# cloneofsimo/paint-with-words-sd

Hardware: NVIDIA H100
Metric: unet_steps_per_sec_512sq_cfg (higher is better)
Workload: dtype f16

## Files before the change

### include/pww_b200.h

```cpp
#ifndef PWW_B200_H_
#define PWW_B200_H_

#include <stddef.h>
#include <stdint.h>

#ifdef __cplusplus
extern "C" {
#endif

typedef enum {
  PWW_OK = 0,
  PWW_ERR_BAD_ARG = -1,
  PWW_ERR_UNSUPPORTED = -2,
  PWW_ERR_CUDA = -3,
  PWW_ERR_WORKSPACE = -4
} pww_status_t;

#define PWW_STAT_MAX 0
#define PWW_STAT_STD 1

int pww_version(void);

const char* pww_status_str(int status);

// ... 45 lines not shown
int pww_xattn_fused_bf16(const void* q, const void* k, const void* v, void* out,
                         int B, int H, int N, int T, int D,
                         int64_t q_batch_stride, int64_t q_row_stride,
                         int64_t k_batch_stride, int64_t k_row_stride,
                         int64_t o_batch_stride, int64_t o_row_stride,
                         const void* mpack, int64_t mpack_batch_stride, int Bw, const int8_t* cidx,
                         const int32_t* wmap_index, int stat, const float* g_sigma, float scale,
                         float* stats, void* workspace, size_t workspace_bytes, void* stream);

int pww_xattn_stats_multi_f16(const void* q, const void* k,
                              int B, int H, int N, int T, int D,
                              int64_t q_batch_stride, int64_t q_row_stride,
                              int64_t k_batch_stride, int64_t k_row_stride,
                              const int32_t* stat, const int32_t* wmap_index,
                              float* stats ,
                              void* workspace, size_t workspace_bytes, void* stream);
int pww_xattn_fwd_multi_f16(const void* q, const void* k, const void* v, void* out,
                            int B, int H, int N, int T, int D,
                            int64_t q_batch_stride, int64_t q_row_stride,
                            int64_t k_batch_stride, int64_t k_row_stride,
                            int64_t o_batch_stride, int64_t o_row_stride,
                            const float* wmap, int64_t wmap_batch_stride, const int32_t* wmap_index,
                            const float* stats, const float* g_sigma, float scale, void* stream);
int pww_xattn_fused_multi_f16(const void* q, const void* k, const void* v, void* out,
                              int B, int H, int N, int T, int D,
                              int64_t q_batch_stride, int64_t q_row_stride,
                              int64_t k_batch_stride, int64_t k_row_stride,
                              int64_t o_batch_stride, int64_t o_row_stride,
                              const void* mpack, int64_t mpack_batch_stride, int Bw, const int8_t* cidx,
                              const int32_t* wmap_index, const int32_t* stat, const float* g_sigma, float scale,
                              float* stats, void* workspace, size_t workspace_bytes, void* stream);
int pww_xattn_stats_multi_bf16(const void* q, const void* k,
                               int B, int H, int N, int T, int D,
                               int64_t q_batch_stride, int64_t q_row_stride,
                               int64_t k_batch_stride, int64_t k_row_stride,
                               const int32_t* stat, const int32_t* wmap_index,
                               float* stats ,
                               void* workspace, size_t workspace_bytes, void* stream);
int pww_xattn_fwd_multi_bf16(const void* q, const void* k, const void* v, void* out,
                             int B, int H, int N, int T, int D,
                             int64_t q_batch_stride, int64_t q_row_stride,
                             int64_t k_batch_stride, int64_t k_row_stride,
                             int64_t o_batch_stride, int64_t o_row_stride,
                             const float* wmap, int64_t wmap_batch_stride, const int32_t* wmap_index,
                             const float* stats, const float* g_sigma, float scale, void* stream);
int pww_xattn_fused_multi_bf16(const void* q, const void* k, const void* v, void* out,
                               int B, int H, int N, int T, int D,
                               int64_t q_batch_stride, int64_t q_row_stride,
                               int64_t k_batch_stride, int64_t k_row_stride,
                               int64_t o_batch_stride, int64_t o_row_stride,
                               const void* mpack, int64_t mpack_batch_stride, int Bw, const int8_t* cidx,
                               const int32_t* wmap_index, const int32_t* stat, const float* g_sigma, float scale,
                               float* stats, void* workspace, size_t workspace_bytes, void* stream);

int pww_xattn_fused_rec_f16(const void* q, const void* k, const void* v, void* out,
                            int B, int H, int N, int T, int D,
                            int64_t q_batch_stride, int64_t q_row_stride,
                            int64_t k_batch_stride, int64_t k_row_stride,
                            int64_t o_batch_stride, int64_t o_row_stride,
                            const void* mpack, int64_t mpack_batch_stride, int Bw, const int8_t* cidx,
                            const int32_t* wmap_index, const int32_t* stat, const float* g_sigma, float scale,
                            float* stats, void* workspace, size_t workspace_bytes, void* stream,
                            const int8_t* ridx, const int32_t* rec_index, float* rec_acc, int64_t rec_batch_stride);
int pww_xattn_fused_rec_bf16(const void* q, const void* k, const void* v, void* out,
                             int B, int H, int N, int T, int D,
                             int64_t q_batch_stride, int64_t q_row_stride,
                             int64_t k_batch_stride, int64_t k_row_stride,
                             int64_t o_batch_stride, int64_t o_row_stride,
                             const void* mpack, int64_t mpack_batch_stride, int Bw, const int8_t* cidx,
                             const int32_t* wmap_index, const int32_t* stat, const float* g_sigma, float scale,
                             float* stats, void* workspace, size_t workspace_bytes, void* stream,
                             const int8_t* ridx, const int32_t* rec_index, float* rec_acc, int64_t rec_batch_stride);

int pww_attn_fwd_f16(const void* q, const void* k, const void* v, void* out,
                     int B, int H, int N, int D,
                     int64_t qkv_batch_stride, int64_t qkv_row_stride,
                     int64_t o_batch_stride, int64_t o_row_stride,
                     float scale, void* stream);
int pww_attn_fwd_bf16(const void* q, const void* k, const void* v, void* out,
                      int B, int H, int N, int D,
                      int64_t qkv_batch_stride, int64_t qkv_row_stride,
                      int64_t o_batch_stride, int64_t o_row_stride,
                      float scale, void* stream);

size_t pww_groupnorm_workspace_bytes(int B, int HW, int G);
int pww_groupnorm_nhwc_f16(const void* x, const void* add, int64_t add_batch_stride ,
                           const void* gamma, const void* beta, void* y,
                           int B, int HW, int C, int G, float eps, int silu,
                           void* workspace, size_t workspace_bytes, void* stream);
int pww_groupnorm_nhwc_bf16(const void* x, const void* add, int64_t add_batch_stride ,
                            const void* gamma, const void* beta, void* y,
                            int B, int HW, int C, int G, float eps, int silu,
                            void* workspace, size_t workspace_bytes, void* stream);

int pww_geglu_f16(const void* in, void* out, int64_t M, int I, void* stream);
int pww_geglu_bf16(const void* in, void* out, int64_t M, int I, void* stream);

int pww_add_layernorm_f16(const void* x, const void* res, const void* gamma, const void* beta, void* sum_out, void* y,
                          int64_t M, int C, float eps, void* stream);
int pww_add_layernorm_bf16(const void* x, const void* res, const void* gamma, const void* beta, void* sum_out, void* y,
                           int64_t M, int C, float eps, void* stream);

int pww_resnet_residual_f16(const void* a, const void* h, const float* bias, void* out, int64_t rows, int C,
                            void* stream);
int pww_resnet_residual_bf16(const void* a, const void* h, const float* bias, void* out, int64_t rows, int C,
                             void* stream);

#define PWW_DTYPE_F32 0
#define PWW_DTYPE_F16 1
#define PWW_DTYPE_BF16 4
int pww_sampler_input(const float* latents, const float* scale, const float* extra, void* out, int out_dtype,
                      int m, int channels, int height, int width, void* stream);
int pww_sampler_update(const void* eps, int eps_dtype, int64_t eps_batch_stride, int64_t eps_channel_stride,
                       int64_t eps_row_stride, int64_t eps_col_stride,
                       float* latents, float* history, int history_len, const float* noise,
                       const float* guidance, const float* beta, const float* form,
                       int m, int height, int width, void* stream);

int pww_control_inject_f16(int n, void* const* dst, const void* const* res, const int64_t* elems_per_image, int rows,
                           const float* scales, void* stream);
int pww_control_inject_bf16(int n, void* const* dst, const void* const* res, const int64_t* elems_per_image, int rows,
                            const float* scales, void* stream);

int pww_control_combine_f16(int units, int n, void* const* out, const void* const* res,
                            const int64_t* elems_per_image, int rows, const float* scales, void* stream);
int pww_control_combine_bf16(int units, int n, void* const* out, const void* const* res,
                             const int64_t* elems_per_image, int rows, const float* scales, void* stream);

#ifdef __cplusplus
}
#endif
#endif
```

### paint_with_words_sd_b200/_native.py

```python
from __future__ import annotations

import ctypes
import os
from typing import Optional

import torch

_HERE = os.path.dirname(os.path.abspath(__file__))
LIB_PATH = os.environ.get("PWW_B200_LIB", os.path.join(_HERE, "libpww_b200.so"))

PWW_STAT_MAX, PWW_STAT_STD = 0, 1
PWW_DTYPE_F32, PWW_DTYPE_F16, PWW_DTYPE_BF16 = 0, 1, 4

EXPORTS = (
    "pww_version", "pww_status_str", "pww_last_cuda_error", "pww_device_supported",
    "pww_xattn_workspace_bytes", "pww_xattn_stats_f16", "pww_xattn_fwd_f16", "pww_attn_fwd_f16",
    "pww_xattn_fused_workspace_bytes", "pww_xattn_fused_f16",
    "pww_xattn_stats_multi_f16", "pww_xattn_fwd_multi_f16", "pww_xattn_fused_multi_f16",
    "pww_groupnorm_workspace_bytes", "pww_groupnorm_nhwc_f16", "pww_geglu_f16", "pww_add_layernorm_f16",
    "pww_sampler_input", "pww_sampler_update",
    "pww_xattn_stats_bf16", "pww_xattn_fwd_bf16", "pww_xattn_fused_bf16",
    "pww_xattn_stats_multi_bf16", "pww_xattn_fwd_multi_bf16", "pww_xattn_fused_multi_bf16",
    "pww_attn_fwd_bf16", "pww_groupnorm_nhwc_bf16", "pww_geglu_bf16", "pww_add_layernorm_bf16",
    "pww_control_inject_f16", "pww_control_inject_bf16",
    "pww_control_combine_f16", "pww_control_combine_bf16",
    "pww_resnet_residual_f16", "pww_resnet_residual_bf16",
    "pww_xattn_fused_rec_f16", "pww_xattn_fused_rec_bf16",
)


class NativeError(RuntimeError):
    pass


_lib: Optional[ctypes.CDLL] = None
launch_count = 0


def lib() -> ctypes.CDLL:
    global _lib
    if _lib is not None:
        return _lib
    if not os.path.exists(LIB_PATH):
        raise NativeError(
            f"{LIB_PATH} not found: build it with `python -m paint_with_words_sd_b200.csrc.build` "
            "(there is no CPU / PyTorch fallback for the attention path)")
    L = ctypes.CDLL(LIB_PATH)
    c_i, c_i64, c_vp, c_f, c_sz = ctypes.c_int, ctypes.c_int64, ctypes.c_void_p, ctypes.c_float, ctypes.c_size_t
    L.pww_version.restype = c_i
    L.pww_status_str.restype = ctypes.c_char_p
    L.pww_status_str.argtypes = [c_i]
    L.pww_last_cuda_error.restype = ctypes.c_char_p
    L.pww_device_supported.restype = c_i
    L.pww_xattn_workspace_bytes.restype = c_sz
    L.pww_xattn_workspace_bytes.argtypes = [c_i] * 5
    L.pww_xattn_stats_f16.restype = c_i
    L.pww_xattn_stats_f16.argtypes = [c_vp, c_vp, c_i, c_i, c_i, c_i, c_i, c_i64, c_i64, c_i64, c_i64, c_i, c_vp,
                                      c_vp, c_vp, c_sz, c_vp]
    L.pww_xattn_fwd_f16.restype = c_i
    L.pww_xattn_fwd_f16.argtypes = [c_vp, c_vp, c_vp, c_vp, c_i, c_i, c_i, c_i, c_i, c_i64, c_i64, c_i64, c_i64,
                                    c_i64, c_i64, c_vp, c_i64, c_vp, c_vp, c_vp, c_f, c_vp]
    L.pww_xattn_fused_workspace_bytes.restype = c_sz
    L.pww_xattn_fused_workspace_bytes.argtypes = []
    L.pww_xattn_fused_f16.restype = c_i
    L.pww_xattn_fused_f16.argtypes = [c_vp, c_vp, c_vp, c_vp, c_i, c_i, c_i, c_i, c_i, c_i64, c_i64, c_i64, c_i64,
                                      c_i64, c_i64, c_vp, c_i64, c_i, c_vp, c_vp, c_i, c_vp, c_f, c_vp, c_vp, c_sz, c_vp]
    L.pww_xattn_stats_multi_f16.restype = c_i
    L.pww_xattn_stats_multi_f16.argtypes = [c_vp, c_vp, c_i, c_i, c_i, c_i, c_i, c_i64, c_i64, c_i64, c_i64, c_vp, c_vp,
                                            c_vp, c_vp, c_sz, c_vp]
    L.pww_xattn_fwd_multi_f16.restype = c_i
    L.pww_xattn_fwd_multi_f16.argtypes = list(L.pww_xattn_fwd_f16.argtypes)
    L.pww_xattn_fused_multi_f16.restype = c_i
    L.pww_xattn_fused_multi_f16.argtypes = [c_vp, c_vp, c_vp, c_vp, c_i, c_i, c_i, c_i, c_i, c_i64, c_i64, c_i64, c_i64,
                                            c_i64, c_i64, c_vp, c_i64, c_i, c_vp, c_vp, c_vp, c_vp, c_f, c_vp, c_vp, c_sz,
                                            c_vp]
    L.pww_xattn_fused_rec_f16.restype = c_i
    L.pww_xattn_fused_rec_f16.argtypes = list(L.pww_xattn_fused_multi_f16.argtypes) + [c_vp, c_vp, c_vp, c_i64]
    L.pww_attn_fwd_f16.restype = c_i
    L.pww_attn_fwd_f16.argtypes = [c_vp, c_vp, c_vp, c_vp, c_i, c_i, c_i, c_i, c_i64, c_i64, c_i64, c_i64, c_f, c_vp]
    L.pww_groupnorm_workspace_bytes.restype = c_sz
    L.pww_groupnorm_workspace_bytes.argtypes = [c_i, c_i, c_i]
    L.pww_groupnorm_nhwc_f16.restype = c_i
    L.pww_groupnorm_nhwc_f16.argtypes = [c_vp, c_vp, c_i64, c_vp, c_vp, c_vp, c_i, c_i, c_i, c_i, c_f, c_i, c_vp, c_sz, c_vp]
    L.pww_geglu_f16.restype = c_i
    L.pww_geglu_f16.argtypes = [c_vp, c_vp, c_i64, c_i, c_vp]
    L.pww_add_layernorm_f16.restype = c_i
    L.pww_add_layernorm_f16.argtypes = [c_vp, c_vp, c_vp, c_vp, c_vp, c_vp, c_i64, c_i, c_f, c_vp]
    L.pww_resnet_residual_f16.restype = c_i
    L.pww_resnet_residual_f16.argtypes = [c_vp, c_vp, c_vp, c_vp, c_i64, c_i, c_vp]
    L.pww_control_inject_f16.restype = c_i
    L.pww_control_inject_f16.argtypes = [c_i, ctypes.POINTER(c_vp), ctypes.POINTER(c_vp), ctypes.POINTER(c_i64), c_i,
                                         c_vp, c_vp]
    L.pww_control_combine_f16.restype = c_i
    L.pww_control_combine_f16.argtypes = [c_i, c_i, ctypes.POINTER(c_vp), ctypes.POINTER(c_vp), ctypes.POINTER(c_i64),
                                          c_i, c_vp, c_vp]
    for name in EXPORTS:
        if name.endswith("_bf16"):
            twin = getattr(L, name[:-len("_bf16")] + "_f16")
            fn = getattr(L, name)
            fn.restype, fn.argtypes = twin.restype, list(twin.argtypes)
    L.pww_sampler_input.restype = c_i
    L.pww_sampler_input.argtypes = [c_vp, c_vp, c_vp, c_vp, c_i, c_i, c_i, c_i, c_i, c_vp]
    L.pww_sampler_update.restype = c_i
    L.pww_sampler_update.argtypes = [c_vp, c_i, c_i64, c_i64, c_i64, c_i64, c_vp, c_vp, c_i, c_vp, c_vp, c_vp, c_vp,
                                     c_i, c_i, c_i, c_vp]
    _lib = L
    return L


def entry(name: str, dtype):
    return getattr(lib(), name + ("_bf16" if dtype == torch.bfloat16 else "_f16"))


def check(status: int, what: str) -> None:
    if status != 0:
        L = lib()
        msg = L.pww_status_str(status).decode()
        if status == -3:
            msg += ": " + L.pww_last_cuda_error().decode()
        raise NativeError(f"{what} failed: {msg} (status {status})")
```

### paint_with_words_sd_b200/csrc/mma_sm90.cuh

```cuda
#pragma once
#include <cuda_runtime.h>
#include <stdint.h>

#include <type_traits>

#include "pww_common.cuh"

namespace pww {
namespace ptx {

__device__ __forceinline__ uint32_t smem_u32(const void* p) { return (uint32_t)__cvta_generic_to_shared(p); }

__device__ __forceinline__ void cp_async16(uint32_t dst, const void* src, uint32_t src_bytes) {
  asm volatile("cp.async.cg.shared.global [%0], [%1], 16, %2;" ::"r"(dst), "l"(src), "r"(src_bytes) : "memory");
}
__device__ __forceinline__ void cp_async_commit() { asm volatile("cp.async.commit_group;" ::: "memory"); }
template <int N>
__device__ __forceinline__ void cp_async_wait() { asm volatile("cp.async.wait_group %0;" ::"n"(N) : "memory"); }

__device__ __forceinline__ void ldsm_x4(uint32_t addr, uint32_t& r0, uint32_t& r1, uint32_t& r2, uint32_t& r3) {
  asm volatile("ldmatrix.sync.aligned.m8n8.x4.shared.b16 {%0, %1, %2, %3}, [%4];"
               : "=r"(r0), "=r"(r1), "=r"(r2), "=r"(r3) : "r"(addr));
}
__device__ __forceinline__ void ldsm_x4_t(uint32_t addr, uint32_t& r0, uint32_t& r1, uint32_t& r2, uint32_t& r3) {
  asm volatile("ldmatrix.sync.aligned.m8n8.x4.trans.shared.b16 {%0, %1, %2, %3}, [%4];"
               : "=r"(r0), "=r"(r1), "=r"(r2), "=r"(r3) : "r"(addr));
}
__device__ __forceinline__ void ldsm_x2_t(uint32_t addr, uint32_t& r0, uint32_t& r1) {
  asm volatile("ldmatrix.sync.aligned.m8n8.x2.trans.shared.b16 {%0, %1}, [%2];" : "=r"(r0), "=r"(r1) : "r"(addr));
}

template <typename E>
__device__ __forceinline__ void mma16816(float* c, const uint32_t* a, uint32_t b0, uint32_t b1) {
  static_assert(std::is_same_v<E, __half> || std::is_same_v<E, __nv_bfloat16>, "fp16 or bf16 operands");
  if constexpr (std::is_same_v<E, __half>) {
    asm volatile(
        "mma.sync.aligned.m16n8k16.row.col.f32.f16.f16.f32 {%0, %1, %2, %3}, {%4, %5, %6, %7}, {%8, %9}, "
        "{%0, %1, %2, %3};"
        : "+f"(c[0]), "+f"(c[1]), "+f"(c[2]), "+f"(c[3])
        : "r"(a[0]), "r"(a[1]), "r"(a[2]), "r"(a[3]), "r"(b0), "r"(b1));
  } else {
    asm volatile(
        "mma.sync.aligned.m16n8k16.row.col.f32.bf16.bf16.f32 {%0, %1, %2, %3}, {%4, %5, %6, %7}, {%8, %9}, "
        "{%0, %1, %2, %3};"
        : "+f"(c[0]), "+f"(c[1]), "+f"(c[2]), "+f"(c[3])
        : "r"(a[0]), "r"(a[1]), "r"(a[2]), "r"(a[3]), "r"(b0), "r"(b1));
  }
}

__device__ __forceinline__ float ex2(float x) {
  float y;
  asm("ex2.approx.ftz.f32 %0, %1;" : "=f"(y) : "f"(x));
  return y;
}
template <typename E>
__device__ __forceinline__ uint32_t pack2(float lo, float hi) {
  const typename Elem<E>::E2 h = Elem<E>::from_float2(lo, hi);
  return *reinterpret_cast<const uint32_t*>(&h);
}
template <typename E>
__device__ __forceinline__ float2 unpack2(uint32_t v) {
  return Elem<E>::to_float2(*reinterpret_cast<const typename Elem<E>::E2*>(&v));
}
__device__ __forceinline__ unsigned long long ld_acquire_gpu_u64(const unsigned long long* p) {
  unsigned long long v;
  asm volatile("ld.acquire.gpu.global.u64 %0, [%1];" : "=l"(v) : "l"(p) : "memory");
  return v;
}

}
}
```

### paint_with_words_sd_b200/csrc/pww_abi.cu

```cuda
#include <stdio.h>
#include <string.h>

#include "pww_common.cuh"
#include "xattn_tc.cuh"
#include "xattn_fused2.cuh"
#include "attn_tc.cuh"
#include "unet_ops.cuh"
#include "sampler_step.cuh"
#include "control_inject.cuh"
#include "control_combine.cuh"
#include <stdlib.h>
#include <algorithm>
#include <type_traits>

namespace {

thread_local char g_last_cuda_error[640] = "";

int cuda_fail(cudaError_t e);

bool aligned16(const void* p) { return (reinterpret_cast<uintptr_t>(p) & 15u) == 0; }

bool supported_head_dim(int D) { return D == 40 || D == 64 || D == 80 || D == 160; }

int check_common(const void* q, const void* k, int B, int H, int N, int T, int D, int64_t q_bs, int64_t q_rs,
                 int64_t k_bs, int64_t k_rs) {
  if (!q || !k || B <= 0 || H <= 0 || N <= 0 || T <= 0 || D <= 0) return PWW_ERR_BAD_ARG;
  if (!aligned16(q) || !aligned16(k)) return PWW_ERR_BAD_ARG;
  if ((q_bs | q_rs | k_bs | k_rs) & 7) return PWW_ERR_BAD_ARG;
  if (q_rs < (int64_t)H * D || k_rs < (int64_t)H * D) return PWW_ERR_BAD_ARG;
  if (!supported_head_dim(D) || !pww::core::supported_keys(T)) return PWW_ERR_UNSUPPORTED;
  return PWW_OK;
}

template <int D_, int KC_>
struct Shape {
  static constexpr int D = D_, KC = KC_;
};
template <int D, typename F>
cudaError_t with_chunks(int T, F&& f) {
  switch (pww::core::chunks_of(T)) {
    case 1: return f(Shape<D, 1>{});
    case 2: return f(Shape<D, 2>{});
    case 3: return f(Shape<D, 3>{});
  }
  return cudaErrorInvalidValue;
}
template <typename F>
cudaError_t with_shape(int D, int T, F&& f) {
  switch (D) {
    case 40: return with_chunks<40>(T, f);
    case 64: return with_chunks<64>(T, f);
    case 80: return with_chunks<80>(T, f);
    case 160: return with_chunks<160>(T, f);
  }
  return cudaErrorInvalidValue;
}

template <int lo, int hi, typename F>
void with_int(int v, F&& f) {
  if constexpr (lo < hi)
    if (v != lo) return with_int<lo + 1, hi>(v, f);
  f(std::integral_constant<int, lo>{});
}

size_t align_up(size_t x, size_t a) { return (x + a - 1) / a * a; }

constexpr int kStatSlotsPerImage = 2048;

int cuda_fail(cudaError_t e) {
  snprintf(g_last_cuda_error, sizeof(g_last_cuda_error), "%s: %s ", cudaGetErrorName(e), cudaGetErrorString(e));
  return PWW_ERR_CUDA;
}

template <typename E>
pww::XattnParams<E> xattn_params(const void* q, const void* k, const void* v, void* out, int B, int H, int N, int T, int D,
                                 int64_t q_bs, int64_t q_rs, int64_t k_bs, int64_t k_rs, int64_t o_bs, int64_t o_rs) {
  pww::XattnParams<E> p;
  memset(&p, 0, sizeof(p));
  p.q = (const E*)q; p.k = (const E*)k; p.v = (const E*)v; p.out = (E*)out;
  p.B = B; p.H = H; p.N = N; p.T = T; p.D = D;
  p.q_bs = q_bs; p.q_rs = q_rs; p.k_bs = k_bs; p.k_rs = k_rs; p.o_bs = o_bs; p.o_rs = o_rs;
  return p;
}

template <typename E>
pww::XattnParams<E> images(const pww::XattnParams<E>& p, int b0, int n) {
  pww::XattnParams<E> c = p;
  c.B = n;
// ... 163 lines not shown
  if (!x || !gamma || !beta || !y || !workspace || B <= 0 || HW <= 0 || C <= 0 || G <= 0) return PWW_ERR_BAD_ARG;
  if (!aligned16(x) || !aligned16(y) || !aligned16(gamma) || !aligned16(beta) || (add && !aligned16(add)))
    return PWW_ERR_BAD_ARG;
  if ((C & 7) || (C % G) || G > 64 || (C >> 3) > 1024) return PWW_ERR_UNSUPPORTED;
  if (add && ((add_batch_stride & 7) || add_batch_stride < C)) return PWW_ERR_BAD_ARG;
  if (workspace_bytes < pww_groupnorm_workspace_bytes(B, HW, G)) return PWW_ERR_WORKSPACE;
  const pww::uops::GnSplit sp = pww::uops::gn_split(HW, C, G);
  pww::uops::GnParams<E> p;
  p.x = (const E*)x; p.add = (const E*)add; p.add_bs = add_batch_stride; p.gamma = (const E*)gamma; p.beta = (const E*)beta;
  p.y = (E*)y;
  p.partial = (float2*)workspace;
  p.HW = HW; p.C = C; p.G = G; p.eps = eps; p.silu = silu;
  p.sv = sp.sv; p.chunks = sp.chunks; p.rows_per_chunk = sp.rows_per_chunk;
  cudaStream_t s = (cudaStream_t)stream;
  const size_t smem1 = (64 + (size_t)2 * sp.rpp * sp.sv * 8) * sizeof(float);
  if (smem1 > 48 * 1024) {
    const cudaError_t e = pww::allow_dynamic_smem<pww::uops::gn_stats_kernel<E>>(64 * 1024 + 256);
    if (e != cudaSuccess) return cuda_fail(e);
  }
  pww::uops::gn_stats_kernel<E><<<dim3(sp.chunks, sp.slices, B), sp.threads, smem1, s>>>(p);
  int rows = 4;
  while (rows > 1 && (long long)B * sp.slices * pww::ceil_div(HW, sp.rpp * rows) < 2 * pww::num_sms()) rows >>= 1;
  cudaLaunchAttribute pdl;
  pdl.id = cudaLaunchAttributeProgrammaticStreamSerialization;
  pdl.val.programmaticStreamSerializationAllowed = 1;
  cudaLaunchConfig_t cfg = {};
  cfg.gridDim = dim3(pww::ceil_div(HW, sp.rpp * rows), sp.slices, B);
  cfg.blockDim = dim3(sp.threads);
  cfg.stream = s;
  cfg.attrs = &pdl;
  cfg.numAttrs = 1;
  cudaError_t e = cudaLaunchKernelEx(&cfg, pww::uops::gn_apply_kernel<E>, p, sp.rpp * rows);
  if (e == cudaSuccess) e = cudaGetLastError();
  return e == cudaSuccess ? PWW_OK : cuda_fail(e);
}

template <typename E>
int geglu(const void* in, void* out, int64_t M, int I, void* stream) {
  if (!in || !out || M <= 0 || I <= 0 || !aligned16(in) || !aligned16(out)) return PWW_ERR_BAD_ARG;
  if (I & 7) return PWW_ERR_UNSUPPORTED;
  const long long total = (long long)M * (I >> 3);
  long long blocks = (total + 255) / 256;
  const long long cap = (long long)pww::num_sms() * 16;
  if (blocks > cap) blocks = cap;
  pww::uops::geglu_kernel<E><<<(int)blocks, 256, 0, (cudaStream_t)stream>>>((const E*)in, (E*)out, M, I);
  cudaError_t e = cudaGetLastError();
  return e == cudaSuccess ? PWW_OK : cuda_fail(e);
}

template <typename E>
int add_layernorm(const void* x, const void* res, const void* gamma, const void* beta, void* sum_out, void* y, int64_t M,
                  int C, float eps, void* stream) {
  if (!x || !gamma || !beta || !y || M <= 0 || C <= 0) return PWW_ERR_BAD_ARG;
  if (!aligned16(x) || !aligned16(y) || !aligned16(gamma) || !aligned16(beta) || (res && !aligned16(res)) ||
      (sum_out && !aligned16(sum_out)))
    return PWW_ERR_BAD_ARG;
  if ((C & 7) || C > 2048) return PWW_ERR_UNSUPPORTED;
  const int warps = 8;
  const unsigned grid = (unsigned)((M + warps - 1) / warps);
  with_int<1, 8>(((C >> 3) + 31) / 32, [&](auto vpl) {
    pww::uops::add_layernorm_kernel<E, vpl><<<grid, warps * 32, 0, (cudaStream_t)stream>>>(
        (const E*)x, (const E*)res, (const E*)gamma, (const E*)beta, (E*)sum_out, (E*)y, M, C, eps);
  });
  cudaError_t e = cudaGetLastError();
  return e == cudaSuccess ? PWW_OK : cuda_fail(e);
}

template <typename E>
int resnet_residual(const void* a, const void* h, const float* bias, void* out, int64_t rows, int C, void* stream) {
  if (!a || !h || !bias || !out || rows <= 0 || C <= 0 || (C & 7)) return PWW_ERR_BAD_ARG;
  if (!aligned16(a) || !aligned16(h) || !aligned16(bias) || !aligned16(out)) return PWW_ERR_BAD_ARG;
  const long long total = (long long)rows * (C >> 3);
  long long blocks = (total + 255) / 256;
  const long long cap = (long long)pww::num_sms() * 16;
  if (blocks > cap) blocks = cap;
  pww::uops::resnet_residual_kernel<E><<<(int)blocks, 256, 0, (cudaStream_t)stream>>>(
      (const E*)a, (const E*)h, bias, (E*)out, total, C >> 3);
  cudaError_t e = cudaGetLastError();
  return e == cudaSuccess ? PWW_OK : cuda_fail(e);
}

template <typename E>
int attn_fwd(const void* q,const void* k, const void* v, void* out, int B, int H, int N, int D, int64_t qkv_batch_stride,
             int64_t qkv_row_stride, int64_t o_batch_stride, int64_t o_row_stride, float scale, void* stream) {
  if (!q || !k || !v || !out || B <= 0 || H <= 0 || N <= 0 || D <= 0) return PWW_ERR_BAD_ARG;
  if (!aligned16(q) || !aligned16(k) || !aligned16(v) || !aligned16(out)) return PWW_ERR_BAD_ARG;
  if ((qkv_batch_stride | qkv_row_stride | o_batch_stride | o_row_stride) & 7) return PWW_ERR_BAD_ARG;
  if (qkv_row_stride < (int64_t)H * D || o_row_stride < (int64_t)H * D) return PWW_ERR_BAD_ARG;
  if (!supported_head_dim(D)) return PWW_ERR_UNSUPPORTED;
  const cudaError_t e = with_shape(D, 1, [&](auto sh) {
    return pww::fa::launch<sh.D, E>(q, k, v, out, B, H, N, qkv_batch_stride, qkv_row_stride, o_batch_stride,
                                    o_row_stride, scale, (cudaStream_t)stream);
  });
  return e == cudaSuccess ? PWW_OK : cuda_fail(e);
}

template <typename E>
int control_inject(int n, void* const* dst, const void* const* res, const int64_t* elems_per_image, int rows,
                   const float* scales, void* stream) {
  if (n < 1 || n > pww::ctl::kMaxLevels || rows < 1 || !dst || !res || !elems_per_image) return PWW_ERR_BAD_ARG;
  pww::ctl::InjectArgs a;
  a.off[0] = 0;
  for (int k = 0; k < n; ++k) {
    const int64_t e = elems_per_image[k];
    if (e <= 0 || (e % pww::ctl::kVec) != 0) return PWW_ERR_BAD_ARG;
    if (!dst[k] || !res[k] || !aligned16(dst[k]) || !aligned16(res[k])) return PWW_ERR_BAD_ARG;
    a.dst[k] = dst[k];
    a.res[k] = res[k];
    a.vec_per_image[k] = e / pww::ctl::kVec;
    a.off[k + 1] = a.off[k] + (int64_t)rows * a.vec_per_image[k];
  }
  for (int k = n; k < pww::ctl::kMaxLevels; ++k) {
    a.dst[k] = nullptr;
    a.res[k] = nullptr;
    a.vec_per_image[k] = 0;
    a.off[k + 1] = a.off[n];
  }
  a.scales = scales;
  a.n = n;
  a.rows = rows;
  const cudaError_t e = pww::ctl::launch_inject<E>(a, (int64_t)pww::num_sms() * 8, (cudaStream_t)stream);
  return e == cudaSuccess ? PWW_OK : cuda_fail(e);
}

template <typename E>
int control_combine(int units, int n, void* const* out, const void* const* res, const int64_t* elems_per_image,
                    int rows, const float* scales, void* stream) {
  if (units < 1 || units > pww::ctl::kMaxUnits || n < 1 || n > pww::ctl::kMaxLevels || rows < 1 || !out || !res ||
      !elems_per_image || !scales)
    return PWW_ERR_BAD_ARG;
  pww::ctl::CombineArgs a = {};
  for (int k = 0; k < n; ++k) {
    const int64_t e = elems_per_image[k];
    if (e <= 0 || (e % pww::ctl::kVec) != 0) return PWW_ERR_BAD_ARG;
    if (!out[k] || !aligned16(out[k])) return PWW_ERR_BAD_ARG;
    a.out[k] = out[k];
    a.vec_per_image[k] = e / pww::ctl::kVec;
    a.off[k + 1] = a.off[k] + (int64_t)rows * a.vec_per_image[k];
  }
  for (int i = 0; i < units * n; ++i) {
    if (!res[i] || !aligned16(res[i])) return PWW_ERR_BAD_ARG;
    a.res[i] = res[i];
  }
  for (int k = n; k < pww::ctl::kMaxLevels; ++k) a.off[k + 1] = a.off[n];
  a.scales = scales;
  a.units = units;
  a.n = n;
  a.rows = rows;
  const cudaError_t e = pww::ctl::launch_combine<E>(a, (int64_t)pww::num_sms() * 8, (cudaStream_t)stream);
  return e == cudaSuccess ? PWW_OK : cuda_fail(e);
}

}

extern "C" {

int pww_xattn_stats_f16(const void* q, const void* k, int B, int H, int N, int T, int D, int64_t q_batch_stride,
    int64_t q_row_stride, int64_t k_batch_stride, int64_t k_row_stride, int stat, const int32_t* wmap_index,
    float* stats, void* workspace, size_t workspace_bytes, void* stream) {
  return xattn_stats<__half>(
      q, k, B, H, N, T, D, q_batch_stride, q_row_stride, k_batch_stride, k_row_stride, stat, nullptr, false,
      wmap_index, stats, workspace, workspace_bytes, stream);
}
int pww_xattn_stats_bf16(const void* q, const void* k, int B, int H, int N, int T, int D, int64_t q_batch_stride,
    int64_t q_row_stride, int64_t k_batch_stride, int64_t k_row_stride, int stat, const int32_t* wmap_index,
    float* stats, void* workspace, size_t workspace_bytes, void* stream) {
  return xattn_stats<__nv_bfloat16>(
      q, k, B, H, N, T, D, q_batch_stride, q_row_stride, k_batch_stride, k_row_stride, stat, nullptr, false,
      wmap_index, stats, workspace, workspace_bytes, stream);
}

int pww_xattn_stats_multi_f16(const void* q, const void* k, int B, int H, int N, int T, int D, int64_t q_batch_stride,
// ... 40 lines not shown
    const float* g_sigma, float scale, void* stream) {
  return xattn_fwd<__nv_bfloat16>(
      q, k, v, out, B, H, N, T, D, q_batch_stride, q_row_stride, k_batch_stride, k_row_stride,
      o_batch_stride, o_row_stride, wmap, wmap_batch_stride, wmap_index, stats, g_sigma, 1, scale, stream);
}

size_t pww_xattn_fused_workspace_bytes(void) { return pww::fx::fused_workspace_bytes(); }

int pww_xattn_fused_f16(const void* q, const void* k, const void* v, void* out, int B, int H, int N, int T, int D,
    int64_t q_batch_stride, int64_t q_row_stride, int64_t k_batch_stride, int64_t k_row_stride, int64_t o_batch_stride,
    int64_t o_row_stride, const void* mpack, int64_t mpack_batch_stride, int Bw, const int8_t* cidx,
    const int32_t* wmap_index, int stat, const float* g_sigma, float scale, float* stats, void* workspace,
    size_t workspace_bytes, void* stream) {
  return xattn_fused<__half>(q, k, v, out, B, H, N, T, D, q_batch_stride, q_row_stride, k_batch_stride, k_row_stride,
      o_batch_stride, o_row_stride, mpack, mpack_batch_stride, Bw, cidx, wmap_index, stat, nullptr, false,
      g_sigma, scale, stats, workspace, workspace_bytes, stream);
}
int pww_xattn_fused_bf16(const void* q, const void* k, const void* v, void* out, int B, int H, int N, int T, int D,
    int64_t q_batch_stride, int64_t q_row_stride, int64_t k_batch_stride, int64_t k_row_stride, int64_t o_batch_stride,
    int64_t o_row_stride, const void* mpack, int64_t mpack_batch_stride, int Bw, const int8_t* cidx,
    const int32_t* wmap_index, int stat, const float* g_sigma, float scale, float* stats, void* workspace,
    size_t workspace_bytes, void* stream) {
  return xattn_fused<__nv_bfloat16>(
      q, k, v, out, B, H, N, T, D, q_batch_stride, q_row_stride, k_batch_stride, k_row_stride,
      o_batch_stride, o_row_stride, mpack, mpack_batch_stride, Bw, cidx, wmap_index, stat, nullptr, false,
      g_sigma, scale, stats, workspace, workspace_bytes, stream);
}

int pww_xattn_fused_multi_f16(const void* q, const void* k, const void* v, void* out, int B, int H, int N, int T, int D,
    int64_t q_batch_stride, int64_t q_row_stride, int64_t k_batch_stride, int64_t k_row_stride, int64_t o_batch_stride,
    int64_t o_row_stride, const void* mpack, int64_t mpack_batch_stride, int Bw, const int8_t* cidx,
    const int32_t* wmap_index, const int32_t* stat, const float* g_sigma, float scale, float* stats, void* workspace,
    size_t workspace_bytes, void* stream) {
  return xattn_fused<__half>(q, k, v, out, B, H, N, T, D, q_batch_stride, q_row_stride, k_batch_stride, k_row_stride,
      o_batch_stride, o_row_stride, mpack, mpack_batch_stride, Bw, cidx, wmap_index, PWW_STAT_MAX, stat, true,
      g_sigma, scale, stats, workspace, workspace_bytes, stream);
}
int pww_xattn_fused_multi_bf16(const void* q, const void* k, const void* v, void* out, int B, int H, int N, int T, int D,
    int64_t q_batch_stride, int64_t q_row_stride, int64_t k_batch_stride, int64_t k_row_stride, int64_t o_batch_stride,
    int64_t o_row_stride, const void* mpack, int64_t mpack_batch_stride, int Bw, const int8_t* cidx,
    const int32_t* wmap_index, const int32_t* stat, const float* g_sigma, float scale, float* stats, void* workspace,
    size_t workspace_bytes, void* stream) {
  return xattn_fused<__nv_bfloat16>(
      q, k, v, out, B, H, N, T, D, q_batch_stride, q_row_stride, k_batch_stride, k_row_stride,
      o_batch_stride, o_row_stride, mpack, mpack_batch_stride, Bw, cidx, wmap_index, PWW_STAT_MAX, stat, true,
      g_sigma, scale, stats, workspace, workspace_bytes, stream);
}

int pww_xattn_fused_rec_f16(const void* q, const void* k, const void* v, void* out, int B, int H, int N, int T, int D,
    int64_t q_batch_stride, int64_t q_row_stride, int64_t k_batch_stride, int64_t k_row_stride, int64_t o_batch_stride,
    int64_t o_row_stride, const void* mpack, int64_t mpack_batch_stride, int Bw, const int8_t* cidx,
    const int32_t* wmap_index, const int32_t* stat, const float* g_sigma, float scale, float* stats, void* workspace,
    size_t workspace_bytes, void* stream, const int8_t* ridx, const int32_t* rec_index, float* rec_acc,
    int64_t rec_batch_stride) {
  const pww::fx::FxRecord rec = {ridx, rec_index, rec_acc, rec_batch_stride};
  return xattn_fused<__half>(q, k, v, out, B, H, N, T, D, q_batch_stride, q_row_stride, k_batch_stride, k_row_stride,
      o_batch_stride, o_row_stride, mpack, mpack_batch_stride, Bw, cidx, wmap_index, PWW_STAT_MAX, stat, true,
      g_sigma, scale, stats, workspace, workspace_bytes, stream, &rec);
}
int pww_xattn_fused_rec_bf16(const void* q, const void* k, const void* v, void* out, int B, int H, int N, int T, int D,
    int64_t q_batch_stride, int64_t q_row_stride, int64_t k_batch_stride, int64_t k_row_stride, int64_t o_batch_stride,
    int64_t o_row_stride, const void* mpack, int64_t mpack_batch_stride, int Bw, const int8_t* cidx,
    const int32_t* wmap_index, const int32_t* stat, const float* g_sigma, float scale, float* stats, void* workspace,
    size_t workspace_bytes, void* stream, const int8_t* ridx, const int32_t* rec_index, float* rec_acc,
    int64_t rec_batch_stride) {
  const pww::fx::FxRecord rec = {ridx, rec_index, rec_acc, rec_batch_stride};
  return xattn_fused<__nv_bfloat16>(
      q, k, v, out, B, H, N, T, D, q_batch_stride, q_row_stride, k_batch_stride, k_row_stride,
      o_batch_stride, o_row_stride, mpack, mpack_batch_stride, Bw, cidx, wmap_index, PWW_STAT_MAX, stat, true,
      g_sigma, scale, stats, workspace, workspace_bytes, stream, &rec);
}

int pww_attn_fwd_f16(const void* q, const void* k, const void* v, void* out, int B, int H, int N, int D,
    int64_t qkv_batch_stride, int64_t qkv_row_stride, int64_t o_batch_stride, int64_t o_row_stride, float scale,
    void* stream) {
  return attn_fwd<__half>(
      q, k, v, out, B, H, N, D, qkv_batch_stride, qkv_row_stride, o_batch_stride, o_row_stride, scale, stream);
}
int pww_attn_fwd_bf16(const void* q, const void* k, const void* v, void* out, int B, int H, int N, int D,
    int64_t qkv_batch_stride, int64_t qkv_row_stride, int64_t o_batch_stride, int64_t o_row_stride, float scale,
    void* stream) {
  return attn_fwd<__nv_bfloat16>(
      q, k, v, out, B, H, N, D, qkv_batch_stride, qkv_row_stride, o_batch_stride, o_row_stride, scale, stream);
}

size_t pww_groupnorm_workspace_bytes(int B, int HW, int G) {
  if (B <= 0 || HW <= 0 || G <= 0) return 0;
  const size_t chunks = (size_t)std::min(HW, pww::uops::kGnMaxChunks);
  return align_up((size_t)B * G * chunks * sizeof(float2), 256);
}

int pww_groupnorm_nhwc_f16(const void* x, const void* add, int64_t add_batch_stride, const void* gamma,
    const void* beta, void* y, int B, int HW, int C, int G, float eps, int silu, void* workspace, size_t workspace_bytes,
    void* stream) {
  return groupnorm_nhwc<__half>(
      x, add, add_batch_stride, gamma, beta, y, B, HW, C, G, eps, silu, workspace, workspace_bytes,
      stream);
}
int pww_groupnorm_nhwc_bf16(const void* x, const void* add, int64_t add_batch_stride, const void* gamma,
    const void* beta, void* y, int B, int HW, int C, int G, float eps, int silu, void* workspace, size_t workspace_bytes,
    void* stream) {
  return groupnorm_nhwc<__nv_bfloat16>(
      x, add, add_batch_stride, gamma, beta, y, B, HW, C, G, eps, silu, workspace, workspace_bytes,
      stream);
}

int pww_geglu_f16(const void* in, void* out, int64_t M, int I, void* stream) {
  return geglu<__half>(in, out, M, I, stream);
}
int pww_geglu_bf16(const void* in, void* out, int64_t M, int I, void* stream) {
  return geglu<__nv_bfloat16>(in, out, M, I, stream);
}

int pww_add_layernorm_f16(const void* x, const void* res, const void* gamma, const void* beta, void* sum_out, void* y,
    int64_t M, int C, float eps, void* stream) {
  return add_layernorm<__half>(x, res, gamma, beta, sum_out, y, M, C, eps, stream);
}
int pww_add_layernorm_bf16(const void* x, const void* res, const void* gamma, const void* beta, void* sum_out, void* y,
    int64_t M, int C, float eps, void* stream) {
  return add_layernorm<__nv_bfloat16>(x, res, gamma, beta, sum_out, y, M, C, eps, stream);
}

int pww_resnet_residual_f16(const void* a, const void* h, const float* bias, void* out, int64_t rows, int C,
                            void* stream) {
  return resnet_residual<__half>(a, h, bias, out, rows, C, stream);
}
int pww_resnet_residual_bf16(const void* a, const void* h, const float* bias, void* out, int64_t rows, int C,
                             void* stream) {
  return resnet_residual<__nv_bfloat16>(a, h, bias, out, rows, C, stream);
}

int pww_sampler_input(const float* latents, const float* scale, const float* extra, void* out, int out_dtype, int m,
                      int channels, int height, int width, void* stream) {
  if (!latents || !scale || !out || m <= 0 || height <= 0 || width <= 0) return PWW_ERR_BAD_ARG;
  if (channels != 4 && channels != 9) return PWW_ERR_BAD_ARG;
  if ((channels == 9) != (extra != nullptr)) return PWW_ERR_BAD_ARG;
  if (out_dtype != PWW_DTYPE_F32 && out_dtype != PWW_DTYPE_F16 && out_dtype != PWW_DTYPE_BF16) return PWW_ERR_UNSUPPORTED;
  pww::smp::InputArgs a;
  a.lat = latents; a.scale = scale; a.extra = extra; a.out = out; a.m = m; a.C = channels; a.hw = height * width;
  const bool px4 = (a.hw % 4) == 0 && aligned16(latents) && (!extra || aligned16(extra)) && aligned16(out);
  cudaStream_t s = (cudaStream_t)stream;
  const cudaError_t e = out_dtype == PWW_DTYPE_F16    ? pww::smp::launch_input<__half>(a, px4, s)
                        : out_dtype == PWW_DTYPE_BF16 ? pww::smp::launch_input<__nv_bfloat16>(a, px4, s)
                                                      : pww::smp::launch_input<float>(a, px4, s);
  return e == cudaSuccess ? PWW_OK : cuda_fail(e);
}

int pww_sampler_update(const void* eps, int eps_dtype, int64_t eps_batch_stride, int64_t eps_channel_stride,
                       int64_t eps_row_stride, int64_t eps_col_stride, float* latents, float* history, int history_len,
                       const float* noise, const float* guidance, const float* beta, const float* form, int m,
                       int height, int width, void* stream) {
  if (!eps || !latents || !history || !guidance || !beta || !form) return PWW_ERR_BAD_ARG;
  if (m <= 0 || height <= 0 || width <= 0 || history_len < 1 || history_len > 4) return PWW_ERR_BAD_ARG;
  if (eps_dtype != PWW_DTYPE_F32 && eps_dtype != PWW_DTYPE_F16 && eps_dtype != PWW_DTYPE_BF16) return PWW_ERR_UNSUPPORTED;
  pww::smp::UpdateArgs a;
  a.eps = eps; a.e_sn = eps_batch_stride; a.e_sc = eps_channel_stride; a.e_sh = eps_row_stride; a.e_sw = eps_col_stride;
  a.lat = latents; a.hist = history; a.noise = noise; a.gscale = guidance; a.beta = beta; a.form = form;
  a.m = m; a.h = height; a.w = width; a.nh = history_len;
  const int64_t hw = (int64_t)height * width;
  const size_t es = eps_dtype == PWW_DTYPE_F32 ? 4 : 2;
  const bool px4 = (hw % 4) == 0 && aligned16(latents) && aligned16(history) && (!noise || aligned16(noise));
  const size_t need = px4 ? 16 : 4 * es;
  const bool cl = eps_channel_stride == 1 && eps_col_stride == 4 && eps_row_stride == 4 * (int64_t)width &&
                  (reinterpret_cast<uintptr_t>(eps) % need) == 0 && ((size_t)eps_batch_stride * es) % need == 0;
  cudaStream_t s = (cudaStream_t)stream;
  const cudaError_t e = eps_dtype == PWW_DTYPE_F16    ? pww::smp::launch_update<__half>(a, px4, cl, s)
// ... 48 lines not shown
```

Baseline: 159.8.

## Add Hopper wgmma flash-attention kernel for head dim 40 self-attention

Adds an SM90 self-attention kernel that uses warpgroup wgmma for QK^T (shared-memory operands) and for PV (register operands), with a 3-stage cp.async K/V pipeline. Each CTA runs two warpgroups handling 128 query rows. An extra padded chunk whose V column is set to one makes the PV product also produce the softmax row sum. The kernel is the default for D=40, and the old mma.sync path stays reachable through new _mma entry points. The goal is higher tensor-core throughput for the 64x64 UNet self-attention. The risk is that D=40 pads K to 48 and wastes MMA work, and every wgmma is waited on synchronously, so MMA work does not overlap with softmax.

```diff
diff --git a/include/pww_b200.h b/include/pww_b200.h
--- a/include/pww_b200.h
+++ b/include/pww_b200.h
@@ -151,6 +151,16 @@
                       int64_t qkv_batch_stride, int64_t qkv_row_stride,
                       int64_t o_batch_stride, int64_t o_row_stride,
                       float scale, void* stream);
+int pww_attn_fwd_mma_f16(const void* q, const void* k, const void* v, void* out,
+                         int B, int H, int N, int D,
+                         int64_t qkv_batch_stride, int64_t qkv_row_stride,
+                         int64_t o_batch_stride, int64_t o_row_stride,
+                         float scale, void* stream);
+int pww_attn_fwd_mma_bf16(const void* q, const void* k, const void* v, void* out,
+                          int B, int H, int N, int D,
+                          int64_t qkv_batch_stride, int64_t qkv_row_stride,
+                          int64_t o_batch_stride, int64_t o_row_stride,
+                          float scale, void* stream);
 
 size_t pww_groupnorm_workspace_bytes(int B, int HW, int G);
 int pww_groupnorm_nhwc_f16(const void* x, const void* add, int64_t add_batch_stride ,
diff --git a/paint_with_words_sd_b200/_native.py b/paint_with_words_sd_b200/_native.py
--- a/paint_with_words_sd_b200/_native.py
+++ b/paint_with_words_sd_b200/_native.py
@@ -26,6 +26,7 @@
     "pww_control_combine_f16", "pww_control_combine_bf16",
     "pww_resnet_residual_f16", "pww_resnet_residual_bf16",
     "pww_xattn_fused_rec_f16", "pww_xattn_fused_rec_bf16",
+    "pww_attn_fwd_mma_f16", "pww_attn_fwd_mma_bf16",
 )
 
 
@@ -78,6 +79,8 @@
     L.pww_xattn_fused_rec_f16.argtypes = list(L.pww_xattn_fused_multi_f16.argtypes) + [c_vp, c_vp, c_vp, c_i64]
     L.pww_attn_fwd_f16.restype = c_i
     L.pww_attn_fwd_f16.argtypes = [c_vp, c_vp, c_vp, c_vp, c_i, c_i, c_i, c_i, c_i64, c_i64, c_i64, c_i64, c_f, c_vp]
+    L.pww_attn_fwd_mma_f16.restype = c_i
+    L.pww_attn_fwd_mma_f16.argtypes = list(L.pww_attn_fwd_f16.argtypes)
     L.pww_groupnorm_workspace_bytes.restype = c_sz
     L.pww_groupnorm_workspace_bytes.argtypes = [c_i, c_i, c_i]
     L.pww_groupnorm_nhwc_f16.restype = c_i
diff --git a/paint_with_words_sd_b200/csrc/attn_wgmma.cuh b/paint_with_words_sd_b200/csrc/attn_wgmma.cuh
--- /dev/null
+++ b/paint_with_words_sd_b200/csrc/attn_wgmma.cuh
@@ -0,0 +1,199 @@
+#pragma once
+#include "attn_tc.cuh"
+#include "mma_sm90.cuh"
+#include "pww_common.cuh"
+
+namespace pww {
+namespace fa90 {
+
+constexpr int kD = 40;
+constexpr int kDataChunks = kD / 8;
+constexpr int kChunks = kDataChunks + 1;
+constexpr int kWarpgroups = 2;
+constexpr int kThreads = kWarpgroups * 128;
+constexpr int kBM = 64 * kWarpgroups;
+constexpr int kBN = 128;
+constexpr int kStages = 3;
+static_assert(kBM == kBN, "Q, K and V tiles share one shape");
+constexpr uint32_t kSlab = kBN * 16;
+constexpr uint32_t kTileBytes = kChunks * kSlab;
+constexpr uint32_t kOffKV = kTileBytes;
+constexpr uint32_t kSmem = kTileBytes + kStages * 2 * kTileBytes;
+static_assert(2 * kSmem <= 232448, "two CTAs per SM");
+
+constexpr int kPieces = kBN * kDataChunks;
+constexpr int kSlots = (kPieces + kThreads - 1) / kThreads;
+struct Pieces {
+  uint32_t soff[kSlots];
+  int64_t goff[kSlots];
+};
+
+__device__ __forceinline__ Pieces make_pieces(int64_t rs) {
+  Pieces pc;
+#pragma unroll
+  for (int i = 0; i < kSlots; ++i) {
+    const int idx = threadIdx.x + i * kThreads, r = idx / kDataChunks, c = idx - r * kDataChunks;
+    pc.soff[i] = c * kSlab + r * 16;
+    pc.goff[i] = r * rs + c * 8;
+  }
+  return pc;
+}
+
+template <typename E>
+__device__ __forceinline__ void load_tile(const Pieces& pc, uint32_t dst, const E* src, int valid) {
+#pragma unroll
+  for (int i = 0; i < kSlots; ++i) {
+    if (i == kSlots - 1 && threadIdx.x + i * kThreads >= kPieces) break;
+    const bool ok = (int)((pc.soff[i] & (kSlab - 1)) >> 4) < valid;
+    ptx::cp_async16(dst + pc.soff[i], ok ? (const void*)(src + pc.goff[i]) : (const void*)src, ok ? 16u : 0u);
+  }
+}
+
+template <typename E>
+__global__ void __launch_bounds__(kThreads, 2) attn_fwd_wgmma_kernel(const fa::Params<E> p) {
+  extern __shared__ __align__(128) unsigned char smem[];
+  const uint32_t smem0 = ptx::smem_u32(smem);
+  const int tid = threadIdx.x, wg = tid >> 7, warp = tid >> 5, lane = tid & 31;
+  const int qtiles = (p.N + kBM - 1) / kBM;
+  const int bh = blockIdx.x / qtiles, qt = blockIdx.x - bh * qtiles;
+  const int b = bh / p.H, h = bh - b * p.H;
+  const int row_base = qt * kBM;
+  const int64_t head = (int64_t)b * p.bs + h * kD;
+  const int ntiles = (p.N + kBN - 1) / kBN;
+
+  {
+    const uint32_t one = std::is_same_v<E, __half> ? 0x3C00u : 0x3F80u;
+    for (int i = tid; i < (1 + 2 * kStages) * kBN; i += kThreads) {
+      const int t = i / kBN, r = i - t * kBN;
+      const uint32_t tile = t == 0 ? 0u : kOffKV + (uint32_t)(t - 1) * kTileBytes;
+      const bool is_v = t > 0 && ((t - 1) & 1);
+      *reinterpret_cast<uint4*>(smem + tile + kDataChunks * kSlab + r * 16) = make_uint4(is_v ? one : 0u, 0u, 0u, 0u);
+    }
+  }
+  const Pieces pc = make_pieces(p.rs);
+  auto issue_kv = [&](int j) {
+    if (j < ntiles) {
+      const uint32_t st = smem0 + kOffKV + (uint32_t)(j % kStages) * 2 * kTileBytes;
+      const int rows = p.N - j * kBN < kBN ? p.N - j * kBN : kBN;
+      load_tile(pc, st, p.k + head + (int64_t)j * kBN * p.rs, rows);
+      load_tile(pc, st + kTileBytes, p.v + head + (int64_t)j * kBN * p.rs, rows);
+    }
+    ptx::cp_async_commit();
+  };
+  load_tile(pc, smem0, p.q + head + (int64_t)row_base * p.rs, p.N - row_base < kBM ? p.N - row_base : kBM);
+  issue_kv(0);
+  issue_kv(1);
+
+  float o[24];
+#pragma unroll
+  for (int i = 0; i < 24; ++i) o[i] = 0.f;
+  float m0 = -INFINITY, m1 = -INFINITY;
+  const float sl2 = p.scale * 1.4426950408889634f;
+  const uint32_t qs = smem0 + (uint32_t)wg * 64 * 16;
+#pragma unroll 1
+  for (int jt = 0; jt < ntiles; ++jt) {
+    ptx::cp_async_wait<1>();
+    ptx::fence_proxy_async();
+    __syncthreads();
+    issue_kv(jt + 2);
+    const uint32_t ks = smem0 + kOffKV + (uint32_t)(jt % kStages) * 2 * kTileBytes, vs = ks + kTileBytes;
+
+    float s[64];
+    ptx::wgmma_fence();
+    ptx::wgmma_m64n128k16_ss<E, false>(s, ptx::gmma_desc(qs, kSlab, 16 * 8), ptx::gmma_desc(ks, kSlab, 16 * 8));
+#pragma unroll
+    for (int kk = 1; kk < 3; ++kk)
+      ptx::wgmma_m64n128k16_ss<E, true>(s, ptx::gmma_desc(qs + kk * 2 * kSlab, kSlab, 16 * 8),
+                                        ptx::gmma_desc(ks + kk * 2 * kSlab, kSlab, 16 * 8));
+    ptx::wgmma_commit();
+    ptx::wgmma_wait<0>();
+#pragma unroll
+    for (int i = 0; i < 64; ++i) ptx::reg_fence(s[i]);
+
+    const int kv = p.N - jt * kBN;
+    if (kv < kBN) {
+#pragma unroll
+      for (int i = 0; i < 64; ++i)
+        if (8 * (i >> 2) + 2 * (lane & 3) + (i & 1) >= kv) s[i] = -INFINITY;
+    }
+    float t0 = -INFINITY, t1 = -INFINITY;
+#pragma unroll
+    for (int j = 0; j < 16; ++j) {
+      t0 = fmaxf(t0, fmaxf(s[4 * j], s[4 * j + 1]));
+      t1 = fmaxf(t1, fmaxf(s[4 * j + 2], s[4 * j + 3]));
+    }
+    t0 = fmaxf(t0, __shfl_xor_sync(0xffffffffu, t0, 1));
+    t0 = fmaxf(t0, __shfl_xor_sync(0xffffffffu, t0, 2));
+    t1 = fmaxf(t1, __shfl_xor_sync(0xffffffffu, t1, 1));
+    t1 = fmaxf(t1, __shfl_xor_sync(0xffffffffu, t1, 2));
+    const float mn0 = fmaxf(m0, t0), mn1 = fmaxf(m1, t1);
+    const float a0 = ptx::ex2((m0 - mn0) * sl2), a1 = ptx::ex2((m1 - mn1) * sl2);
+    m0 = mn0; m1 = mn1;
+    const float n0 = -mn0 * sl2, n1 = -mn1 * sl2;
+    uint32_t pa[8][4];
+#pragma unroll
+    for (int j = 0; j < 16; ++j) {
+      pa[j >> 1][(j & 1) * 2] = ptx::pack2<E>(ptx::ex2(fmaf(s[4 * j], sl2, n0)), ptx::ex2(fmaf(s[4 * j + 1], sl2, n0)));
+      pa[j >> 1][(j & 1) * 2 + 1] =
+          ptx::pack2<E>(ptx::ex2(fmaf(s[4 * j + 2], sl2, n1)), ptx::ex2(fmaf(s[4 * j + 3], sl2, n1)));
+    }
+#pragma unroll
+    for (int j = 0; j < 6; ++j) {
+      o[4 * j] *= a0; o[4 * j + 1] *= a0; o[4 * j + 2] *= a1; o[4 * j + 3] *= a1;
+    }
+#pragma unroll
+    for (int i = 0; i < 24; ++i) ptx::reg_fence(o[i]);
+#pragma unroll
+    for (int kk = 0; kk < 8; ++kk)
+#pragma unroll
+      for (int e = 0; e < 4; ++e) ptx::reg_fence(pa[kk][e]);
+    ptx::wgmma_fence();
+#pragma unroll
+    for (int kk = 0; kk < 8; ++kk)
+      ptx::wgmma_m64n48k16_rs<E>(o, pa[kk], ptx::gmma_desc(vs + kk * 2 * 128, 128, kSlab));
+    ptx::wgmma_commit();
+    ptx::wgmma_wait<0>();
+#pragma unroll
+    for (int i = 0; i < 24; ++i) ptx::reg_fence(o[i]);
+#pragma unroll
+    for (int kk = 0; kk < 8; ++kk)
+#pragma unroll
+      for (int e = 0; e < 4; ++e) ptx::reg_fence(pa[kk][e]);
+  }
+
+  const float i0 = 1.f / __shfl_sync(0xffffffffu, o[20], lane & ~3);
+  const float i1 = 1.f / __shfl_sync(0xffffffffu, o[22], lane & ~3);
+  __syncthreads();
+  const int g = lane >> 2, q = lane & 3, r0 = warp * 16 + g;
+#pragma unroll
+  for (int j = 0; j < kDataChunks; ++j) {
+    *reinterpret_cast<uint32_t*>(smem + j * kSlab + r0 * 16 + q * 4) = ptx::pack2<E>(o[4 * j] * i0, o[4 * j + 1] * i0);
+    *reinterpret_cast<uint32_t*>(smem + j * kSlab + (r0 + 8) * 16 + q * 4) =
+        ptx::pack2<E>(o[4 * j + 2] * i1, o[4 * j + 3] * i1);
+  }
+  __syncwarp();
+  E* ob = p.out + (int64_t)b * p.o_bs + h * kD;
+  for (int idx = lane; idx < 16 * kDataChunks; idx += 32) {
+    const int r = idx / kDataChunks, c = idx - r * kDataChunks, row = row_base + warp * 16 + r;
+    if (row < p.N)
+      *reinterpret_cast<uint4*>(ob + (int64_t)row * p.o_rs + c * 8) =
+          *reinterpret_cast<const uint4*>(smem + c * kSlab + (warp * 16 + r) * 16);
+  }
+}
+
+template <typename E>
+cudaError_t launch(const void* q, const void* k, const void* v, void* out, int B, int H, int N, int64_t bs, int64_t rs,
+                   int64_t o_bs, int64_t o_rs, float scale, cudaStream_t s) {
+  fa::Params<E> p;
+  p.q = (const E*)q; p.k = (const E*)k; p.v = (const E*)v; p.out = (E*)out;
+  p.B = B; p.H = H; p.N = N; p.bs = bs; p.rs = rs; p.o_bs = o_bs; p.o_rs = o_rs; p.scale = scale;
+  const cudaError_t e = allow_dynamic_smem<attn_fwd_wgmma_kernel<E>>(kSmem);
+  if (e != cudaSuccess) return e;
+  const long long grid = (long long)B * H * ((N + kBM - 1) / kBM);
+  if (grid > 0x7fffffffLL) return cudaErrorInvalidConfiguration;
+  attn_fwd_wgmma_kernel<E><<<(unsigned)grid, kThreads, kSmem, s>>>(p);
+  return cudaGetLastError();
+}
+
+}
+}
diff --git a/paint_with_words_sd_b200/csrc/mma_sm90.cuh b/paint_with_words_sd_b200/csrc/mma_sm90.cuh
--- a/paint_with_words_sd_b200/csrc/mma_sm90.cuh
+++ b/paint_with_words_sd_b200/csrc/mma_sm90.cuh
@@ -48,6 +48,55 @@
   }
 }
 
+__device__ __forceinline__ uint64_t gmma_desc(uint32_t smem_addr, uint32_t lbo, uint32_t sbo) {
+  return (uint64_t)((smem_addr & 0x3FFFFu) >> 4) | ((uint64_t)((lbo >> 4) & 0x3FFFu) << 16) |
+         ((uint64_t)((sbo >> 4) & 0x3FFFu) << 32);
+}
+__device__ __forceinline__ void fence_proxy_async() { asm volatile("fence.proxy.async.shared::cta;" ::: "memory"); }
+__device__ __forceinline__ void wgmma_fence() { asm volatile("wgmma.fence.sync.aligned;" ::: "memory"); }
+__device__ __forceinline__ void wgmma_commit() { asm volatile("wgmma.commit_group.sync.aligned;" ::: "memory"); }
+template <int N>
+__device__ __forceinline__ void wgmma_wait() { asm volatile("wgmma.wait_group.sync.aligned %0;" ::"n"(N) : "memory"); }
+__device__ __forceinline__ void reg_fence(float& r) { asm volatile("" : "+f"(r)::"memory"); }
+__device__ __forceinline__ void reg_fence(uint32_t& r) { asm volatile("" : "+r"(r)::"memory"); }
+
+#define PWW_ACC8(c, i) c(d[i]), c(d[i + 1]), c(d[i + 2]), c(d[i + 3]), c(d[i + 4]), c(d[i + 5]), c(d[i + 6]), c(d[i + 7])
+#define PWW_ACC24(c) PWW_ACC8(c, 0), PWW_ACC8(c, 8), PWW_ACC8(c, 16)
+#define PWW_ACC64(c) PWW_ACC24(c), PWW_ACC8(c, 24), PWW_ACC8(c, 32), PWW_ACC8(c, 40), PWW_ACC8(c, 48), PWW_ACC8(c, 56)
+#define PWW_R24 "%0, %1, %2, %3, %4, %5, %6, %7, %8, %9, %10, %11, %12, %13, %14, %15, %16, %17, %18, %19, %20, %21, %22, %23"
+#define PWW_R64                                                                                                         \
+  PWW_R24 ", %24, %25, %26, %27, %28, %29, %30, %31, %32, %33, %34, %35, %36, %37, %38, %39, %40, %41, %42, %43, %44, " \
+          "%45, %46, %47, %48, %49, %50, %51, %52, %53, %54, %55, %56, %57, %58, %59, %60, %61, %62, %63"
+#define PWW_WGMMA_N128_SS(TY, SCALE_D, C)                                                                          \
+  asm volatile("{\n.reg .pred p;\nsetp.ne.b32 p, %66, 0;\n"                                                        \
+               "wgmma.mma_async.sync.aligned.m64n128k16.f32" TY " {" PWW_R64 "}, %64, %65, p, 1, 1, 0, 0;\n}\n"  \
+               : PWW_ACC64(C) : "l"(da), "l"(db), "n"(SCALE_D))
+template <typename E, bool ACC>
+__device__ __forceinline__ void wgmma_m64n128k16_ss(float (&d)[64], uint64_t da, uint64_t db) {
+  static_assert(std::is_same_v<E, __half> || std::is_same_v<E, __nv_bfloat16>, "fp16 or bf16 operands");
+  if constexpr (std::is_same_v<E, __half>) {
+    if constexpr (ACC) PWW_WGMMA_N128_SS(".f16.f16", 1, "+f"); else PWW_WGMMA_N128_SS(".f16.f16", 0, "=f");
+  } else {
+    if constexpr (ACC) PWW_WGMMA_N128_SS(".bf16.bf16", 1, "+f"); else PWW_WGMMA_N128_SS(".bf16.bf16", 0, "=f");
+  }
+}
+#define PWW_WGMMA_N48_RS(TY)                                                                                           \
+  asm volatile("{\n.reg .pred p;\nsetp.ne.b32 p, %29, 0;\n"                                                           \
+               "wgmma.mma_async.sync.aligned.m64n48k16.f32" TY " {" PWW_R24 "}, {%24, %25, %26, %27}, %28, p, 1, 1, 1;\n}\n" \
+               : PWW_ACC24("+f") : "r"(a[0]), "r"(a[1]), "r"(a[2]), "r"(a[3]), "l"(db), "n"(1))
+template <typename E>
+__device__ __forceinline__ void wgmma_m64n48k16_rs(float (&d)[24], const uint32_t (&a)[4], uint64_t db) {
+  static_assert(std::is_same_v<E, __half> || std::is_same_v<E, __nv_bfloat16>, "fp16 or bf16 operands");
+  if constexpr (std::is_same_v<E, __half>) PWW_WGMMA_N48_RS(".f16.f16"); else PWW_WGMMA_N48_RS(".bf16.bf16");
+}
+#undef PWW_WGMMA_N48_RS
+#undef PWW_WGMMA_N128_SS
+#undef PWW_R64
+#undef PWW_R24
+#undef PWW_ACC64
+#undef PWW_ACC24
+#undef PWW_ACC8
+
 __device__ __forceinline__ float ex2(float x) {
   float y;
   asm("ex2.approx.ftz.f32 %0, %1;" : "=f"(y) : "f"(x));
diff --git a/paint_with_words_sd_b200/csrc/pww_abi.cu b/paint_with_words_sd_b200/csrc/pww_abi.cu
--- a/paint_with_words_sd_b200/csrc/pww_abi.cu
+++ b/paint_with_words_sd_b200/csrc/pww_abi.cu
@@ -5,6 +5,7 @@
 #include "xattn_tc.cuh"
 #include "xattn_fused2.cuh"
 #include "attn_tc.cuh"
+#include "attn_wgmma.cuh"
 #include "unet_ops.cuh"
 #include "sampler_step.cuh"
 #include "control_inject.cuh"
@@ -334,12 +335,18 @@
 
 template <typename E>
 int attn_fwd(const void* q,const void* k, const void* v, void* out, int B, int H, int N, int D, int64_t qkv_batch_stride,
-             int64_t qkv_row_stride, int64_t o_batch_stride, int64_t o_row_stride, float scale, void* stream) {
+             int64_t qkv_row_stride, int64_t o_batch_stride, int64_t o_row_stride, float scale, void* stream,
+             bool mma_sync = false) {
   if (!q || !k || !v || !out || B <= 0 || H <= 0 || N <= 0 || D <= 0) return PWW_ERR_BAD_ARG;
   if (!aligned16(q) || !aligned16(k) || !aligned16(v) || !aligned16(out)) return PWW_ERR_BAD_ARG;
   if ((qkv_batch_stride | qkv_row_stride | o_batch_stride | o_row_stride) & 7) return PWW_ERR_BAD_ARG;
   if (qkv_row_stride < (int64_t)H * D || o_row_stride < (int64_t)H * D) return PWW_ERR_BAD_ARG;
   if (!supported_head_dim(D)) return PWW_ERR_UNSUPPORTED;
+  if (D == pww::fa90::kD && !mma_sync) {
+    const cudaError_t e = pww::fa90::launch<E>(q, k, v, out, B, H, N, qkv_batch_stride, qkv_row_stride, o_batch_stride,
+                                               o_row_stride, scale, (cudaStream_t)stream);
+    return e == cudaSuccess ? PWW_OK : cuda_fail(e);
+  }
   const cudaError_t e = with_shape(D, 1, [&](auto sh) {
     return pww::fa::launch<sh.D, E>(q, k, v, out, B, H, N, qkv_batch_stride, qkv_row_stride, o_batch_stride,
                                     o_row_stride, scale, (cudaStream_t)stream);
@@ -546,6 +553,18 @@
     void* stream) {
   return attn_fwd<__nv_bfloat16>(
       q, k, v, out, B, H, N, D, qkv_batch_stride, qkv_row_stride, o_batch_stride, o_row_stride, scale, stream);
+}
+int pww_attn_fwd_mma_f16(const void* q, const void* k, const void* v, void* out, int B, int H, int N, int D,
+    int64_t qkv_batch_stride, int64_t qkv_row_stride, int64_t o_batch_stride, int64_t o_row_stride, float scale,
+    void* stream) {
+  return attn_fwd<__half>(
+      q, k, v, out, B, H, N, D, qkv_batch_stride, qkv_row_stride, o_batch_stride, o_row_stride, scale, stream, true);
+}
+int pww_attn_fwd_mma_bf16(const void* q, const void* k, const void* v, void* out, int B, int H, int N, int D,
+    int64_t qkv_batch_stride, int64_t qkv_row_stride, int64_t o_batch_stride, int64_t o_row_stride, float scale,
+    void* stream) {
+  return attn_fwd<__nv_bfloat16>(
+      q, k, v, out, B, H, N, D, qkv_batch_stride, qkv_row_stride, o_batch_stride, o_row_stride, scale, stream, true);
 }
 
 size_t pww_groupnorm_workspace_bytes(int B, int HW, int G) {
```

Result: no change. 161.2 (median of 6 runs) (+0.9%).
